# HKUST-Aerial-Robotics/A-LOAM

Hardware: AMD Instinct MI355X
Metric: HDL-64 scans/sec (whole node) (higher is better)
Workload: dtype f32 features / f64 solve

## Files before the change

a-loam_amd/csrc/aloam_device.hpp:

```cpp
#pragma once
#include <hip/hip_runtime.h>
#include <stdint.h>
#include "aloam_atan.hpp"

namespace aloam {

constexpr int kFrontSlots = 128 + 8;
constexpr int kBlockPts = 1024;
constexpr int kMaxRings = 128;
constexpr int kSectors = 6;
constexpr int kSharpPerSector = 2;
constexpr int kLessSharpPerSector = 20;
constexpr int kFlatPerSector = 4;
constexpr int kSharpPerRing = kSectors * kSharpPerSector;
constexpr int kLessSharpPerRing = kSectors * kLessSharpPerSector;
constexpr int kFlatPerRing = kSectors * kFlatPerSector;
constexpr int kNnTile = 1024;

enum ErrBits { kErrEmpty = 1, kErrRingCap = 2, kErrPointCap = 4, kErrInternal = 8 };

struct alignas(16) SeqMeta {
  int n_in;
  int first_kept, last_kept;
  int half_idx;
  float start_ori, end_ori;
  int n_cloud;
  int err;
  int n_sharp, n_less_sharp, n_flat, n_less_flat;
  int n_corner_last, n_surf_last;
  int parity;
  int pad1;
};

struct alignas(16) OdomState {
  double para_q[4];
  double para_t[3];
  double q_w[4];
  double t_w[3];
  int corner_corr[2], plane_corr[2];
  int lm_iterations[2], lm_successful[2];
  double initial_cost[2], final_cost[2];
  int termination[2];
  int inited;
  int pad;
};

enum SeqBits { kSeqActive = 1, kSeqSolve = 2, kSeqMapGrow = 4 };
__device__ __forceinline__ bool seq_idle(const int* active, int b, int bit = kSeqActive) { return active && !(active[b] & bit); }

struct EdgeRec { float cp[3], a[3], b[3]; int valid; int pad[2]; };
struct PlaneRec { float cp[3], j[3], l[3], m[3]; int valid; int pad[3]; };

struct RegArgs {
  const char* in;
  long long seq_stride;
  int pt_stride;
  int B, cap, R, NB;
  int ring_from_field;
  float min_range;
  SeqMeta* meta;
  float4* slabs;
  int slab;
  unsigned long long* front_lb;
  int* front_ticket;
  int* ringstart;
  float4* cloud;
  float* curv;
  int8_t* label;
  unsigned long long* lookback;
  unsigned epoch;
  int* ring_ticket;
  int store_debug;
  float4* sharp;
  float4* less_sharp[2];
  float4* flat;
  float4* less_flat[2];
  const int* active;
};

constexpr int kRangeRowTables = 6;
struct RangeArgs {
  const int* n_cols;
  const float2* az_xy;
  const float* row_tab;
  int rows, n_az, row_major;
  float range_scale;
};

struct OdomArgs {
  int B, cap, R;
  SeqMeta* meta;
  OdomState* state;
  const float4* sharp;
  const float4* flat;
  const float4* less_sharp[2];
  const float4* less_flat[2];
  const int* active;
  float4* grid_sorted3[2][2];
  float4* grid_sorted2[2][2];
  int* grid_start3[2][2];
  int* grid_start2[2][2];
  float4* grid_sorted3c[2][2];
  int* grid_start3c[2][2];
  int* grid_flags[2][2];
  int* grid_walk[2][2];
  int grid_H_corner, grid_H_surf;
  float4* sel_sharp;
  float4* sel_flat;
  EdgeRec* edges;
  PlaneRec* planes;
  int outer;
  int last_outer;
  int lm_max_iterations;
  int distortion;
};

template <typename T>
__device__ __forceinline__ T* row_of(T* const (&buf)[2], int k, int b, long long per) { return (k ? buf[1] : buf[0]) + b * per; }
__device__ __forceinline__ const float4* corner_last(const OdomArgs& a, int b, int parity) { return row_of(a.less_sharp, parity ^ 1, b, (long long)a.R * kLessSharpPerRing); }
__device__ __forceinline__ const float4* surf_last(const OdomArgs& a, int b, int parity) { return row_of(a.less_flat, parity ^ 1, b, (long long)a.cap); }

struct GridView {
  int H;
  float4 *sorted3, *sorted2, *sorted3c;
  int *start3, *start2, *start3c, *flags, *walk;
};
template <typename T>
__device__ __forceinline__ T* grid_ptr(T* const (&buf)[2][2], int set, int which) {
  return set ? (which ? buf[1][1] : buf[1][0]) : (which ? buf[0][1] : buf[0][0]);
}
__device__ __forceinline__ GridView grid_view(const OdomArgs& a, int b, int which, int set) {
  GridView g;
  g.H = which == 0 ? a.grid_H_corner : a.grid_H_surf;
  const long long per = which == 0 ? (long long)a.R * kLessSharpPerRing : (long long)a.cap;
  g.sorted3 = grid_ptr(a.grid_sorted3, set, which) + b * per;
  g.sorted2 = grid_ptr(a.grid_sorted2, set, which) + b * per;
  g.start3 = grid_ptr(a.grid_start3, set, which) + (long long)b * (g.H + 1);
  g.start2 = grid_ptr(a.grid_start2, set, which) + (long long)b * (g.H + 1);
  g.sorted3c = grid_ptr(a.grid_sorted3c, set, which) + b * per;
  g.start3c = grid_ptr(a.grid_start3c, set, which) + (long long)b * (g.H + 1);
  g.flags = grid_ptr(a.grid_flags, set, which) + b * 4;
  g.walk = grid_ptr(a.grid_walk, set, which) + (long long)b * 2 * (a.R + 8);
  return g;
}

__device__ __forceinline__ float4 load_point(const char* base, long long i, int stride) {
  const float* p = reinterpret_cast<const float*>(base + i * (long long)stride);
  if ((stride & 15) == 0) return *reinterpret_cast<const float4*>(p);
  if (stride == 12) return make_float4(p[0], p[1], p[2], 0.f);
  return make_float4(p[0], p[1], p[2], p[3]);
}

__device__ __forceinline__ bool point_kept(const float4& p, float thres) {
  if (!(isfinite(p.x) && isfinite(p.y) && isfinite(p.z))) return false;
  const float r2 = p.x * p.x + p.y * p.y + p.z * p.z;
  return !(r2 < thres * thres);
}

__device__ __forceinline__ double shfl_down_f64(double v, int d) {
  int lo = __double2loint(v), hi = __double2hiint(v);
  lo = __shfl_down(lo, d, 64);
  hi = __shfl_down(hi, d, 64);
  return __hiloint2double(hi, lo);
}

template <int D>
__device__ __forceinline__ unsigned xor_lane_u32(unsigned v, int lane) {
  if constexpr (D == 1) return (unsigned)__builtin_amdgcn_mov_dpp((int)v, 0xB1, 0xF, 0xF, true);
  else if constexpr (D == 2) return (unsigned)__builtin_amdgcn_mov_dpp((int)v, 0x4E, 0xF, 0xF, true);
  else {
    const unsigned up = (unsigned)__builtin_amdgcn_mov_dpp((int)v, 0x100 + D, 0xF, 0xF, true);
    const unsigned dn = (unsigned)__builtin_amdgcn_mov_dpp((int)v, 0x110 + D, 0xF, 0xF, true);
    return (lane & D) ? dn : up;
  }
}
template <int D, bool MAX>
__device__ __forceinline__ unsigned long long row_step_u64(unsigned long long v, int lane) {
  const unsigned lo = xor_lane_u32<D>((unsigned)v, lane), hi = xor_lane_u32<D>((unsigned)(v >> 32), lane);
  const unsigned long long o = ((unsigned long long)hi << 32) | lo;
  return MAX ? (o > v ? o : v) : (o < v ? o : v);
}
template <bool MAX>
__device__ __forceinline__ unsigned long long wave_extreme_u64(unsigned long long v, int lane) {
  v = row_step_u64<1, MAX>(v, lane);
  v = row_step_u64<2, MAX>(v, lane);
  v = row_step_u64<4, MAX>(v, lane);
  v = row_step_u64<8, MAX>(v, lane);
  unsigned long long best = MAX ? 0ull : ~0ull;
#pragma unroll
  for (int q = 0; q < 4; ++q) {
    const unsigned lo = (unsigned)__builtin_amdgcn_readlane((int)(unsigned)v, 16 * q), hi = (unsigned)__builtin_amdgcn_readlane((int)(unsigned)(v >> 32), 16 * q);
    const unsigned long long o = ((unsigned long long)hi << 32) | lo;
    best = MAX ? (o > best ? o : best) : (o < best ? o : best);
  }
  return best;
}

template <bool MAX>
__device__ __forceinline__ unsigned wave_reduce_u32(unsigned v) {
  constexpr int identity = MAX ? 0 : -1;
  auto op = [](unsigned a, unsigned b) { return MAX ? (a > b ? a : b) : (a < b ? a : b); };
  v = op(v, (unsigned)__builtin_amdgcn_update_dpp(identity, (int)v, 0x111, 0xF, 0xF, false));
  v = op(v, (unsigned)__builtin_amdgcn_update_dpp(identity, (int)v, 0x112, 0xF, 0xF, false));
  v = op(v, (unsigned)__builtin_amdgcn_update_dpp(identity, (int)v, 0x114, 0xF, 0xF, false));
  v = op(v, (unsigned)__builtin_amdgcn_update_dpp(identity, (int)v, 0x118, 0xF, 0xF, false));
  v = op(v, (unsigned)__builtin_amdgcn_update_dpp(identity, (int)v, 0x142, 0xA, 0xF, false));
  v = op(v, (unsigned)__builtin_amdgcn_update_dpp(identity, (int)v, 0x143, 0xC, 0xF, false));
  return (unsigned)__builtin_amdgcn_readlane((int)v, 63);
}
__device__ __forceinline__ unsigned long long wave_min_packed(unsigned long long v) {
  const unsigned hi = (unsigned)(v >> 32), lo = (unsigned)v;
  const unsigned mh = wave_reduce_u32<false>(hi);
  const unsigned long long tie = __ballot(hi == mh);
  unsigned ml;
  if (__popcll(tie) == 1) ml = (unsigned)__builtin_amdgcn_readlane((int)lo, __ffsll((long long)tie) - 1);
  else ml = wave_reduce_u32<false>(hi == mh ? lo : 0xffffffffu);
  return ((unsigned long long)mh << 32) | ml;
}

template <bool MAX>
__device__ __forceinline__ int wave_scan_i32(int v) {
  constexpr int identity = MAX ? (int)0x80000000 : 0;
  auto op = [](int a, int b) { return MAX ? (a > b ? a : b) : a + b; };
  v = op(v, __builtin_amdgcn_update_dpp(identity, v, 0x111, 0xF, 0xF, false));
  v = op(v, __builtin_amdgcn_update_dpp(identity, v, 0x112, 0xF, 0xF, false));
  v = op(v, __builtin_amdgcn_update_dpp(identity, v, 0x114, 0xF, 0xF, false));
  v = op(v, __builtin_amdgcn_update_dpp(identity, v, 0x118, 0xF, 0xF, false));
  v = op(v, __builtin_amdgcn_update_dpp(identity, v, 0x142, 0xA, 0xF, false));
  v = op(v, __builtin_amdgcn_update_dpp(identity, v, 0x143, 0xC, 0xF, false));
  return v;
}

template <typename T, int NT>
__device__ __forceinline__ T block_exclusive_scan(T v, T* lds, T* total) {
  const int tid = threadIdx.x;
  lds[tid] = v;
  __syncthreads();
  for (int d = 1; d < NT; d <<= 1) {
    const T add = tid >= d ? lds[tid - d] : T(0);
    __syncthreads();
    lds[tid] += add;
    __syncthreads();
  }
  const T incl = lds[tid];
  *total = lds[NT - 1];
  __syncthreads();
  return incl - v;
}

__device__ __forceinline__ void wave_box_reduce(float (&mn)[3], float (&mx)[3]) {
#pragma unroll
  for (int q = 0; q < 3; ++q)
    for (int d = 32; d > 0; d >>= 1) { mn[q] = fminf(mn[q], __shfl_down(mn[q], d, 64)); mx[q] = fmaxf(mx[q], __shfl_down(mx[q], d, 64)); }
}

__device__ __forceinline__ int pow2ceil(int v) { int p = 1; while (p < v) p <<= 1; return p; }
template <typename K>
__device__ __forceinline__ void bitonic_cx(K& a, K& b) {
  const K lo = a < b ? a : b, hi = a < b ? b : a;
  a = lo; b = hi;
}
template <bool FIRST, typename K>
__device__ __forceinline__ void bitonic_groups_of_eight(K* keys, int n, int tid) {
  constexpr K kInf = (K)~(K)0;
  for (int g = tid * 8; g < n; g += 2048) {
    K v[8];
#pragma unroll
    for (int u = 0; u < 8; ++u) v[u] = g + u < n ? keys[g + u] : kInf;
    if (FIRST) {
#pragma unroll
      for (int b = 0; b < 8; b += 2) bitonic_cx(v[b], v[b + 1]);
#pragma unroll
      for (int b = 0; b < 8; b += 4) { bitonic_cx(v[b], v[b + 3]); bitonic_cx(v[b + 1], v[b + 2]); }
#pragma unroll
      for (int b = 0; b < 8; b += 2) bitonic_cx(v[b], v[b + 1]);
#pragma unroll
      for (int o = 0; o < 4; ++o) bitonic_cx(v[o], v[7 - o]);
    } else {
#pragma unroll
      for (int o = 0; o < 4; ++o) bitonic_cx(v[o], v[o + 4]);
    }
#pragma unroll
    for (int b = 0; b < 8; b += 4) { bitonic_cx(v[b], v[b + 2]); bitonic_cx(v[b + 1], v[b + 3]); }
#pragma unroll
    for (int b = 0; b < 8; b += 2) bitonic_cx(v[b], v[b + 1]);
#pragma unroll
    for (int u = 0; u < 8; ++u) if (g + u < n) keys[g + u] = v[u];
  }
  __syncthreads();
}
template <typename K>
__device__ __forceinline__ void bitonic_sort_keys(K* keys, int n, int tid) {
  const int npad = pow2ceil(n);
  bitonic_groups_of_eight<true, K>(keys, n, tid);
  for (int k = 16; k <= npad; k <<= 1) {
    const int hk = k >> 1;
    for (int t = tid; t < (npad >> 1); t += 256) {
      const int base = (t / hk) * k, off = t & (hk - 1);
      const int i = base + off, l = base + (k - 1 - off);
      if (l < n) {
        const K x = keys[i], y = keys[l];
        if (x > y) { keys[i] = y; keys[l] = x; }
      }
    }
    __syncthreads();
    for (int j = k >> 2; j > 4; j >>= 1) {
      for (int t = tid; t < (npad >> 1); t += 256) {
        const int i = ((t & ~(j - 1)) << 1) | (t & (j - 1));
        const int l = i + j;
        if (l < n) {
          const K x = keys[i], y = keys[l];
          if (x > y) { keys[i] = y; keys[l] = x; }
        }
      }
      __syncthreads();
    }
    bitonic_groups_of_eight<false, K>(keys, n, tid);
  }
}
__device__ __forceinline__ void bitonic_sort_u64(unsigned long long* keys, int n, int tid) { bitonic_sort_keys<unsigned long long>(keys, n, tid); }


}
```

a-loam_amd/csrc/registration_kernels.hip:

```cpp
#include "aloam_device.hpp"
#include "registration_kernels.hpp"
#include "voxel_device.hpp"

namespace aloam {

struct RecordLoader {
  static constexpr bool kKeepPoint = true;
  const char* in; int stride;
  __device__ __forceinline__ float4 operator()(int i) const { return load_point(in, i, stride); }
};

#ifndef ALOAM_RANGE_KEEP_POINT
#define ALOAM_RANGE_KEEP_POINT 0
#endif
struct RangeLoader {
  static constexpr bool kKeepPoint = ALOAM_RANGE_KEEP_POINT;
  const unsigned short* az; const unsigned short* range;
  const float2* az_xy; const float* tab;
  unsigned div, magic; int n_az; bool row_major; float scale;
  __device__ __forceinline__ float4 operator()(int i) const {
#ifdef ALOAM_RANGE_PHASES
    asm volatile("; ##PHASE decode");
#endif
    const unsigned code = range[i];
    unsigned q = __umulhi((unsigned)i, magic), r = (unsigned)i - q * div;
    if (r >= div) { r -= div; ++q; }
    const int row = (int)(row_major ? q : r), col = (int)(row_major ? r : q);
    const int azc = az[col];
    const bool hit = code != 0u && azc < n_az;
    int ac = azc + reinterpret_cast<const int*>(tab)[4 * kMaxRings + row];
    ac = ac < 0 ? ac + n_az : ac;
    ac = ac >= n_az ? ac - n_az : ac;
    const float2 cs = az_xy[hit ? ac : 0];
    const float rho = (float)code * scale + tab[2 * kMaxRings + row];
    const float rxy = rho * tab[0 * kMaxRings + row];
    const float nan = __builtin_nanf("");
#ifdef ALOAM_RANGE_PHASES
    asm volatile("; ##PHASE body");
#endif
    return make_float4(hit ? rxy * cs.x : nan, hit ? rxy * cs.y : nan, hit ? rho * tab[1 * kMaxRings + row] + tab[3 * kMaxRings + row] : nan, tab[5 * kMaxRings + row]);
  }
};
__device__ __forceinline__ RangeLoader range_loader(const RegArgs& a, const RangeArgs& d, int b, float* tab) {
  for (int q = threadIdx.x; q < kRangeRowTables * kMaxRings; q += blockDim.x) tab[q] = d.row_tab[q];
  __syncthreads();
  const int n_cols = d.n_cols[b];
  const unsigned short* blob = reinterpret_cast<const unsigned short*>(a.in + (long long)b * a.seq_stride);
  const unsigned div = (unsigned)(d.row_major ? n_cols : d.rows);
  return RangeLoader{blob, blob + ((n_cols + 7) & ~7), d.az_xy, tab, div, div ? 0xffffffffu / div : 0u, d.n_az, d.row_major != 0, d.range_scale};
}

template <class Loader>
__device__ __forceinline__ void find_ends_body(const RegArgs& a, const int b, const int n, const Loader& load) {
  const int tid = threadIdx.x;
  __shared__ int s_first, s_last;
  if (tid == 0) { s_first = 0x7fffffff; s_last = -1; }
  __syncthreads();
  for (int base = 0; base < n; base += 4096) {
    bool any = false;
#pragma unroll
    for (int k = 0; k < 4; ++k) {
      const int i = base + k * 1024 + tid;
      if (i < n && point_kept(load(i), a.min_range)) { atomicMin(&s_first, i); any = true; }
    }
    if (__syncthreads_or(any)) break;
  }
  for (int base = 0; base < n; base += 4096) {
    bool any = false;
#pragma unroll
    for (int k = 0; k < 4; ++k) {
      const int i = n - 1 - (base + k * 1024 + tid);
      if (i >= 0 && point_kept(load(i), a.min_range)) { atomicMax(&s_last, i); any = true; }
    }
    if (__syncthreads_or(any)) break;
  }
  __syncthreads();
  if (tid == 0) {
    SeqMeta m = a.meta[b];
    m.n_in = n;
    m.first_kept = s_first;
    m.last_kept = s_last;
    m.half_idx = 0x7fffffff;
    m.err = 0;
    m.n_cloud = 0;
    m.start_ori = 0.f;
    m.end_ori = 0.f;
    if (s_last < 0) {
      m.err = kErrEmpty;
    } else {
      const float4 p0 = load(s_first);
      const float4 p1 = load(s_last);
      const float startOri = -atan2f_port(p0.y, p0.x);
      float endOri = (float)((double)(-atan2f_port(p1.y, p1.x)) + 2 * M_PI);
      if ((double)(endOri - startOri) > 3 * M_PI) endOri = (float)((double)endOri - 2 * M_PI);
      else if ((double)(endOri - startOri) < M_PI) endOri = (float)((double)endOri + 2 * M_PI);
      m.start_ori = startOri;
      m.end_ori = endOri;
    }
    if (n > a.cap) m.err |= kErrPointCap;
    a.meta[b] = m;
  }
}
__global__ __launch_bounds__(1024) void k_find_ends(RegArgs a, const int* __restrict__ n_in) {
  const int b = blockIdx.x;
  if (seq_idle(a.active, b)) return;
  find_ends_body(a, b, n_in[b], RecordLoader{a.in + (long long)b * a.seq_stride, a.pt_stride});
}

__device__ __forceinline__ int ring_from_angle(float angle, int R) {
  int scanID;
  if (R == 16) {
    scanID = (int)((double)((angle + 15) / 2) + 0.5);
    return (scanID > R - 1 || scanID < 0) ? -1 : scanID;
  }
  if (R == 32) {
    scanID = (int)(((double)angle + 92.0 / 3.0) * 3.0 / 4.0);
    return (scanID > R - 1 || scanID < 0) ? -1 : scanID;
  }
  if ((double)angle >= -8.83) scanID = (int)((double)(2 - angle) * 3.0 + 0.5);
  else scanID = R / 2 + (int)((-8.83 - (double)angle) * 2.0 + 0.5);
  if ((double)angle > 2 || (double)angle < -24.33 || scanID > 50 || scanID < 0) return -1;
  return scanID;
}
__device__ __forceinline__ int ring_of(const float4& p, int R, int ring_from_field) {
  if (ring_from_field) {
    const int scanID = (int)p.w;
    return (scanID > R - 1 || scanID < 0) ? -1 : scanID;
  }
  const float s2 = p.x * p.x + p.y * p.y;
  {
    const float t = p.z * __frsqrt_rn(s2), u = t * t;
    const float poly = 1.0f + u * (-0.3333319425582886f + u * (0.19994600117206573f + u * (-0.1420508623123169f + u * (0.10522426664829254f + u * (-0.06763934344053268f + u * 0.025188861414790154f)))));
    const float fast = t * poly * 57.29577951f;
    const int lo = ring_from_angle(fast - 2e-4f, R), hi = ring_from_angle(fast + 2e-4f, R);
    if (lo == hi && fabsf(t) <= 0.65f) return lo;
  }
  const float angle = (float)(atan((double)p.z / sqrt((double)s2)) * 180 / M_PI);
  return ring_from_angle(angle, R);
}

constexpr int kGatherSpinLimit = 1 << 20;
__device__ __forceinline__ void front_publish(unsigned long long* g, unsigned epoch, unsigned prefix, int value) {
  __hip_atomic_store(g, ((unsigned long long)((epoch << 1) | prefix) << 32) | (unsigned)value, __ATOMIC_RELAXED, __HIP_MEMORY_SCOPE_AGENT);
}
template <bool MIN>
__device__ __forceinline__ int front_lookback(unsigned long long* slot0, int blk, unsigned epoch, int local, int* err) {
  constexpr int identity = MIN ? 0x7fffffff : 0;
  unsigned long long* mine = slot0 + (long long)blk * kFrontSlots;
  if (blk == 0) { front_publish(mine, epoch, 1u, local); return identity; }
  front_publish(mine, epoch, 0u, local);
  int acc = identity;
  for (int t = blk - 1; t >= 0; --t) {
    unsigned long long g;
    int spins = 0;
    while ((unsigned)((g = __hip_atomic_load(slot0 + (long long)t * kFrontSlots, __ATOMIC_RELAXED, __HIP_MEMORY_SCOPE_AGENT)) >> 33) != (epoch & 0x7fffffffu)) {
      if (++spins > kGatherSpinLimit) { atomicOr(err, kErrInternal); g = (1ull << 32) | (unsigned)identity; break; }
      __builtin_amdgcn_s_sleep(1);
    }
    const int v = (int)(unsigned)g;
    acc = MIN ? (v < acc ? v : acc) : acc + v;
    if ((g >> 32) & 1ull) break;
  }
  front_publish(mine, epoch, 1u, MIN ? (local < acc ? local : acc) : acc + local);
  return acc;
}

template <bool FIELD_RING, class MakeLoader>
__device__ __forceinline__ void front_body(const RegArgs& a, const MakeLoader& make_loader) {
  const int b = blockIdx.x, tid = threadIdx.x, lane = tid & 63, wave = tid >> 6;
  __shared__ int s_cnt[16][kMaxRings];
  __shared__ int s_half, s_ticket;
  if (seq_idle(a.active, b)) return;
  if (tid == 0) { s_ticket = atomicAdd(a.front_ticket + b, 1); s_half = 0x7fffffff; }
  for (int q = tid; q < 16 * kMaxRings; q += 256) (&s_cnt[0][0])[q] = 0;
  __syncthreads();
  const int blk = s_ticket;
  const SeqMeta m = a.meta[b];
  const int n = m.n_in < a.cap ? m.n_in : a.cap;
  if (blk * kBlockPts >= n) return;
  const auto load = make_loader(b);
  const float startOri = m.start_ori, endOri = m.end_ori;
  int ring[4], rank[4];
  float4 p[4];
  float ori[4];
  int myhalf = 0x7fffffff;
#pragma unroll
  for (int k = 0; k < 4; ++k) {
    const int i = blk * kBlockPts + k * 256 + tid;
    ring[k] = -1;
    p[k] = make_float4(0.f, 0.f, 0.f, 0.f);
    ori[k] = 0.f;
    if (i < n) {
      const float4 q = load(i);
      if (point_kept(q, a.min_range)) {
        ring[k] = ring_of(q, a.R, FIELD_RING ? 1 : a.ring_from_field);
        if (ring[k] >= 0) {
          if constexpr (decltype(load)::kKeepPoint) p[k] = q;
          ori[k] = -atan2f_port(q.y, q.x);
          float o1 = ori[k];
          if ((double)o1 < (double)startOri - M_PI / 2) o1 = (float)((double)o1 + 2 * M_PI);
          else if ((double)o1 > (double)startOri + M_PI * 3 / 2) o1 = (float)((double)o1 - 2 * M_PI);
          if ((double)(o1 - startOri) > M_PI && i < myhalf) myhalf = i;
        }
      }
    }
  }
#pragma unroll
  for (int k = 0; k < 4; ++k) {
    rank[k] = 0;
    unsigned long long todo = __ballot(ring[k] >= 0);
    while (todo) {
      const int leader = __ffsll((long long)todo) - 1;
      const int r = __shfl(ring[k], leader, 64);
      const unsigned long long same = __ballot(ring[k] == r);
      if (ring[k] == r) rank[k] = __popcll(same & ((1ull << lane) - 1ull));
      if (lane == leader) s_cnt[k * 4 + wave][r] = __popcll(same);
      todo &= ~same;
    }
  }
  for (int d = 32; d > 0; d >>= 1) { const int o = __shfl_down(myhalf, d, 64); myhalf = o < myhalf ? o : myhalf; }
  if (lane == 0 && myhalf != 0x7fffffff) atomicMin(&s_half, myhalf);
  __syncthreads();
  unsigned long long* lb = a.front_lb + (long long)b * a.NB * kFrontSlots;
  if (tid < a.R) {
    int total = 0;
#pragma unroll
    for (int q = 0; q < 16; ++q) total += s_cnt[q][tid];
    int run = front_lookback<false>(lb + tid, blk, a.epoch, total, &a.meta[b].err);
#pragma unroll
    for (int q = 0; q < 16; ++q) { const int c = s_cnt[q][tid]; s_cnt[q][tid] = run; run += c; }
  } else if (tid == 192) {
    const int before = front_lookback<true>(lb + a.R, blk, a.epoch, s_half, &a.meta[b].err);
    s_half = before < s_half ? before : s_half;
  }
  __syncthreads();
  const int half_idx = s_half;
  float4* slabs = a.slabs + (long long)b * a.R * a.slab;
#pragma unroll
  for (int k = 0; k < 4; ++k) {
    if (ring[k] < 0) continue;
    const int i = blk * kBlockPts + k * 256 + tid;
    const int pos = s_cnt[k * 4 + wave][ring[k]] + rank[k];
    float o = ori[k];
    if (i <= half_idx) {
      if ((double)o < (double)startOri - M_PI / 2) o = (float)((double)o + 2 * M_PI);
      else if ((double)o > (double)startOri + M_PI * 3 / 2) o = (float)((double)o - 2 * M_PI);
    } else {
      o = (float)((double)o + 2 * M_PI);
      if ((double)o < (double)endOri - M_PI * 3 / 2) o = (float)((double)o + 2 * M_PI);
      else if ((double)o > (double)endOri + M_PI / 2) o = (float)((double)o - 2 * M_PI);
    }
    const float relTime = (o - startOri) / (endOri - startOri);
    const float inten = (float)((double)ring[k] + 0.1 * (double)relTime);
    float4 pk = p[k];
    if constexpr (!decltype(load)::kKeepPoint) pk = load(i);
    if (pos < a.slab) slabs[(long long)ring[k] * a.slab + pos] = make_float4(pk.x, pk.y, pk.z, inten);
  }
}
__global__ __launch_bounds__(256) __attribute__((amdgpu_waves_per_eu(8))) void k_front(RegArgs a) {
  front_body<false>(a, [&](int b) { return RecordLoader{a.in + (long long)b * a.seq_stride, a.pt_stride}; });
}
__global__ __launch_bounds__(64) void k_ring_starts(RegArgs a) {
  const int b = blockIdx.x, lane = threadIdx.x;
  if (seq_idle(a.active, b)) return;
  const int n = a.meta[b].n_in < a.cap ? a.meta[b].n_in : a.cap;
  const int nb = (n + kBlockPts - 1) / kBlockPts;
  const unsigned long long* last = a.front_lb + ((long long)b * a.NB + (nb > 0 ? nb - 1 : 0)) * kFrontSlots;
  int run = 0, err = 0;
  for (int base = 0; base < a.R; base += 64) {
    const int r = base + lane;
    int c = 0;
    if (r < a.R && nb > 0) {
      const unsigned long long g = last[r];
      if ((unsigned)(g >> 32) != (((a.epoch & 0x7fffffffu) << 1) | 1u)) err |= kErrInternal; else c = (int)(unsigned)g;
      if (c > a.slab) { c = a.slab; err |= kErrRingCap; }
    }
    const int inc = wave_scan_i32<false>(c);
    if (r < a.R) a.ringstart[b * (a.R + 1) + r] = run + inc - c;
    run += __builtin_amdgcn_readlane(inc, 63);
  }
  if (err) atomicOr(&a.meta[b].err, err);
  if (lane == 0) {
    a.ringstart[b * (a.R + 1) + a.R] = run;
    a.meta[b].n_cloud = run;
    int half = 0x7fffffff;
    if (nb > 0) { const unsigned long long g = last[a.R]; if ((unsigned)(g >> 32) == (((a.epoch & 0x7fffffffu) << 1) | 1u)) half = (int)(unsigned)g; }
    a.meta[b].half_idx = half;
    a.front_ticket[b] = 0;
  }
}

__global__ __launch_bounds__(256) void k_dense_cloud(RegArgs a) {
  const int r = blockIdx.x, b = blockIdx.y;
  if (seq_idle(a.active, b)) return;
  const int start = a.ringstart[b * (a.R + 1) + r], n = a.ringstart[b * (a.R + 1) + r + 1] - start;
  const float4* src = a.slabs + ((long long)b * a.R + r) * a.slab;
  float4* dst = a.cloud + (long long)b * a.cap + start;
  for (int i = threadIdx.x; i < n; i += 256) dst[i] = src[i];
}

template <bool MAX>
__device__ __forceinline__ unsigned wave_extreme_u32(unsigned v, int lane) { (void)lane; return wave_reduce_u32<MAX>(v); }

__device__ __forceinline__ void publish_count(unsigned long long* slot, unsigned epoch, int count) {
  __hip_atomic_store(slot, ((unsigned long long)epoch << 32) | (unsigned)count, __ATOMIC_RELAXED, __HIP_MEMORY_SCOPE_AGENT);
}
__device__ __forceinline__ int gather_counts(const unsigned long long* slots, int upto, unsigned epoch, int lane, int* err) {
  int sum = 0;
  for (int base = 0; base < upto; base += 64) {
    const int q = base + lane;
    if (q < upto) {
      unsigned long long g;
      int spins = 0;
      while ((unsigned)((g = __hip_atomic_load(slots + q, __ATOMIC_RELAXED, __HIP_MEMORY_SCOPE_AGENT)) >> 32) != epoch) {
        if (++spins > kGatherSpinLimit) { atomicOr(err, kErrInternal); g = 0; break; }
        __builtin_amdgcn_s_sleep(1);
      }
      sum += (int)(unsigned)g;
    }
  }
  sum = wave_scan_i32<false>(sum);
  return __builtin_amdgcn_readlane(sum, 63);
}
constexpr unsigned kCurvThresholdBits = 0x3DCCCCCDu;
constexpr unsigned kInfBits = 0x7f800000u;
template <int K6>
__device__ __forceinline__ void pick_sector(int j, unsigned init_marks, int L, int lane, const float* curv_l, const unsigned char* flags,
                                            short* s_pick, int* s_misc) {
  constexpr int kSlots = kSharpPerSector + kLessSharpPerSector + kFlatPerSector;
  constexpr int NRP = (K6 + 3) / 4;
  const int sp = (L * j) / 6, len = (L * (j + 1)) / 6 - sp;
  const int first = sp + 5;
  typedef unsigned keys_t __attribute__((ext_vector_type(16)));
  static_assert(K6 <= 16, "sector registers");
  keys_t cc;
  unsigned rp[NRP];
#pragma unroll
  for (int q = 0; q < NRP; ++q) rp[q] = 0;
#pragma unroll
  for (int r = 0; r < K6; ++r) {
    const int pos = r * 64 + lane;
    cc[r] = 0u;
    if (pos < len) {
      const int i = first + pos;
      rp[r / 4] |= (unsigned)(flags[i] >> 2) << (8 * (r % 4));
      if (!(pos < 5 && ((init_marks >> pos) & 1u))) cc[r] = __float_as_uint(curv_l[i]) + 1u;
    }
  }
  unsigned spill = 0;
  auto kill = [&](int kr, int f, const unsigned dead) {
    unsigned rb;
    if constexpr (NRP <= 2) {
      const unsigned r0 = (unsigned)__builtin_amdgcn_readlane((int)rp[0], f), r1 = (unsigned)__builtin_amdgcn_readlane((int)rp[NRP - 1], f);
      rb = (unsigned)((((unsigned long long)r1 << 32) | r0) >> (8 * kr));
    } else {
      unsigned rpk = (unsigned)__builtin_amdgcn_readlane((int)rp[0], f);
#pragma unroll
      for (int q = 1; q < NRP; ++q) { const unsigned x = (unsigned)__builtin_amdgcn_readlane((int)rp[q], f); if (q == (kr >> 2)) rpk = x; }
      rb = rpk >> (8 * (kr & 3));
    }
    const int fw = (int)(rb & 7u), bk = (int)((rb >> 3) & 7u);
    const int P = kr * 64 + f;
    const int lo = f - bk, w = fw + bk;
    {
      const bool in = (unsigned)(lane - lo) <= (unsigned)w;
      const unsigned old = cc[kr];
      cc[kr] = in ? dead : old;
    }
    if ((unsigned)lo > (unsigned)(63 - w)) {
      asm volatile("");
      if (lo < 0 && kr > 0) { asm volatile(""); const bool in = lane >= 64 + lo; const unsigned old = cc[kr - 1]; cc[kr - 1] = in ? dead : old; }
      if (lo >= 0 && kr + 1 < K6) { asm volatile(""); const bool in = lane <= lo + w - 64; const unsigned old = cc[kr + 1]; cc[kr + 1] = in ? dead : old; }
    }
    if (P + 5 >= len) {
      asm volatile("");
      const int e = P + fw - (len - 1);
      if (e > 0) spill |= (1u << e) - 1u;
    }
    return P;
  };
  int picks = 0;
  int count = 0;
  for (; count < kLessSharpPerSector; ++count) {
    unsigned m = cc[0];
#pragma unroll
    for (int r = 1; r < K6; ++r) m = cc[r] > m ? cc[r] : m;
    int krl = 0;
#pragma unroll
    for (int r = 1; r < K6; ++r) krl = cc[r] == m ? r : krl;
    const unsigned cmax = wave_reduce_u32<true>(m);
    if (!(cmax - 1u >= kCurvThresholdBits && cmax - 1u <= kInfBits)) break;
    const unsigned long long tie = __ballot(m == cmax);
    int f = __builtin_ctzll(tie);
    int kr = __builtin_amdgcn_readlane(krl, f);
    if (__popcll(tie) != 1) {
      asm volatile("");
      const unsigned w = wave_reduce_u32<true>(m == cmax ? (unsigned)(krl * 64 + lane) : 0u);
      f = (int)(w & 63u); kr = (int)(w >> 6);
    }
    const int P = kill(kr, f, 0u);
    picks = lane == count ? first + P : picks;
  }
  const int ncorner = count;
  if (lane < ncorner) s_pick[j * kSlots + kSharpPerSector + lane] = (short)picks;
#pragma unroll
  for (int r = 0; r < K6; ++r) cc[r] -= 1u;
  count = 0;
  while (true) {
    unsigned m = cc[0];
#pragma unroll
    for (int r = 1; r < K6; ++r) m = cc[r] < m ? cc[r] : m;
    int krl = K6 - 1;
#pragma unroll
    for (int r = K6 - 2; r >= 0; --r) krl = cc[r] == m ? r : krl;
    const unsigned cmin = wave_reduce_u32<false>(m);
    if (!(cmin < kCurvThresholdBits)) break;
    const unsigned long long tie = __ballot(m == cmin);
    int f = __builtin_ctzll(tie);
    int kr = __builtin_amdgcn_readlane(krl, f);
    if (__popcll(tie) != 1) {
      asm volatile("");
      const unsigned w = wave_reduce_u32<false>(m == cmin ? (unsigned)(krl * 64 + lane) : 0xffffffffu);
      f = (int)(w & 63u); kr = (int)(w >> 6);
    }
    picks = lane == count ? first + kr * 64 + f : picks;
    ++count;
    if (count >= kFlatPerSector) break;
    kill(kr, f, 0xffffffffu);
  }
  if (lane < count) s_pick[j * kSlots + kSharpPerSector + kLessSharpPerSector + lane] = (short)picks;
  if (lane == 0) { s_misc[1 + j] = ncorner | (count << 8); s_misc[8 + j] = (int)spill; }
}


#ifdef ALOAM_PHASE_CLOCK
__device__ unsigned long long g_phase_clock[2][32];
constexpr int phase_slot(const char* s) { unsigned h = 0; while (*s) h = h * 33u + (unsigned char)*s++; return (int)(h % 32u); }
#define ALOAM_PHASE(name) do { asm volatile("; ##PHASE " name); if (threadIdx.x == 0) { constexpr int slot_ = phase_slot(name); \
    atomicAdd(&g_phase_clock[0][slot_], (unsigned long long)__builtin_readcyclecounter()); atomicAdd(&g_phase_clock[1][slot_], 1ull); } } while (0)
#else
#define ALOAM_PHASE(name) asm volatile("; ##PHASE " name)
#endif
__device__ __forceinline__ bool label_is_member(unsigned char f) { return ((f + 1u) & 2u) == 0u; }
__device__ __forceinline__ int label_of(unsigned char f) { const int c = f & 3; return c == 3 ? -1 : c; }
template <int NPAD, typename K, int SHIFT>
__device__ __forceinline__ int voxel_runs_tail(unsigned char* smem, unsigned char* flags, int* s_scan, int* s_misc,
                                               const float4* cloud, float4* out, int L, int tid, int lane, int wave,
                                               unsigned long long* lb_lf, int ring, int nrings, unsigned epoch, int* err) {
  const unsigned* vis = reinterpret_cast<const unsigned*>(smem);
  K* rkeys = reinterpret_cast<K*>(smem);
  constexpr unsigned kEMask = SHIFT >= 32 ? 0xffffffffu : ((1u << (SHIFT & 31)) - 1u);
  constexpr int EIT = NPAD / 256;
  unsigned hmask = 0;
  int hrank[EIT];
  unsigned myvi[EIT];
#pragma unroll
  for (int it = 0; it < EIT; ++it) {
    const int e = it * 256 + tid;
    bool h = false;
    myvi[it] = 0xffffffffu;
    if (e < L) {
      const unsigned vi = vis[e];
      const unsigned char fe = flags[e + 5];
      const bool member = label_is_member(fe);
      h = member && (e == 0 || !label_is_member(flags[e + 4]) || vis[e - 1] != vi);
      myvi[it] = vi;
      flags[e + 5] = (unsigned char)((fe & 3u) | (member && !h ? 4u : 0u));
    }
    const unsigned long long m = __ballot(h);
    hrank[it] = __popcll(m & ((1ull << lane) - 1ull));
    if (h) hmask |= 1u << it;
    if (lane == 0) s_scan[it * 4 + wave] = __popcll(m);
  }
  __syncthreads();
  static_assert(4 * EIT <= 64, "one wave scans the table");
  if (wave == 0) {
    const int c = lane < 4 * EIT ? s_scan[lane] : 0;
    const int inc = wave_scan_i32<false>(c);
    if (lane < 4 * EIT) s_scan[lane] = inc - c;
    if (lane == 63) s_scan[64] = inc;
  }
  __syncthreads();
  const int n_runs = s_scan[64];
#pragma unroll
  for (int it = 0; it < EIT; ++it) hrank[it] += s_scan[it * 4 + wave];
#pragma unroll
  for (int it = 0; it < EIT; ++it)
    if ((hmask >> it) & 1u) { const int e = it * 256 + tid; rkeys[hrank[it]] = (K)(((K)myvi[it] << SHIFT) | (K)e); }
  __syncthreads();
  ALOAM_PHASE("after_run_heads");
  bitonic_sort_keys<K>(rkeys, n_runs, tid);

  ALOAM_PHASE("after_sort");
  int n_vox = 0;
  unsigned vmask = 0;
  int vrank[EIT];
  __syncthreads();
#pragma unroll
  for (int it = 0; it < EIT; ++it) {
    const int p = it * 256 + tid;
    const bool h = p < n_runs && (p == 0 || (unsigned)(rkeys[p - 1] >> SHIFT) != (unsigned)(rkeys[p] >> SHIFT));
    const unsigned long long m = __ballot(h);
    vrank[it] = __popcll(m & ((1ull << lane) - 1ull));
    if (h) vmask |= 1u << it;
    if (lane == 0) s_scan[it * 4 + wave] = __popcll(m);
  }
  __syncthreads();
  if (wave == 0) {
    const int c = lane < 4 * EIT ? s_scan[lane] : 0;
    const int inc = wave_scan_i32<false>(c);
    if (lane < 4 * EIT) s_scan[lane] = inc - c;
    if (lane == 63) { s_scan[64] = inc; publish_count(lb_lf + ring, epoch, inc); }
  }
  __syncthreads();
  n_vox = s_scan[64];
#pragma unroll
  for (int it = 0; it < EIT; ++it) vrank[it] += s_scan[it * 4 + wave];
  if (wave == 0) {
    const unsigned long long* lb0 = lb_lf - 3 * nrings;
    const int b0 = gather_counts(lb0 + 0 * nrings, ring, epoch, lane, err), b1 = gather_counts(lb0 + 1 * nrings, ring, epoch, lane, err);
    const int b2 = gather_counts(lb0 + 2 * nrings, ring, epoch, lane, err), b3 = gather_counts(lb_lf, ring, epoch, lane, err);
    if (lane == 0) { s_misc[40] = b0; s_misc[41] = b1; s_misc[42] = b2; s_misc[43] = b3; }
  }
  __syncthreads();
  ALOAM_PHASE("after_vox_heads_gather");
  out += s_misc[43];
#pragma unroll
  for (int it = 0; it < EIT; ++it) {
    if (!((vmask >> it) & 1u)) continue;
    const int p = it * 256 + tid;
    const unsigned vi = (unsigned)(rkeys[p] >> SHIFT);
    voxel::Centroid c;
    for (int q = p; q < n_runs; ++q) {
      const K kq = rkeys[q];
      if ((unsigned)(kq >> SHIFT) != vi) break;
      int e = (int)((unsigned)kq & kEMask);
      bool more;
      do {
        const float4 p0 = cloud[e + 5], p1 = cloud[e + 6], p2 = cloud[e + 7], p3 = cloud[e + 8];
        const bool c1 = e + 1 < L && (flags[e + 6] & 4), c2 = e + 2 < L && (flags[e + 7] & 4), c3 = e + 3 < L && (flags[e + 8] & 4);
        more = e + 4 < L && (flags[e + 9] & 4);
        c.add(p0);
        if (!c1) break;
        c.add(p1);
        if (!c2) break;
        c.add(p2);
        if (!c3) break;
        c.add(p3);
        e += 4;
      } while (more);
    }
    out[vrank[it]] = c.get();
  }
  ALOAM_PHASE("after_centroids");
  return n_vox;
}

template <int NPAD>
__global__ __launch_bounds__(256) __attribute__((amdgpu_waves_per_eu(NPAD <= 2048 ? 8 : 4))) void k_ring_features(RegArgs a, float leaf) {
  constexpr int MAXN = NPAD + 11;
  constexpr int ITEMS = (MAXN + 255) / 256;
  const int b = blockIdx.x, tid = threadIdx.x, lane = tid & 63, wave = tid >> 6;
  extern __shared__ __attribute__((aligned(16))) unsigned char smem_ticket[];
  int* s_ticket = reinterpret_cast<int*>(smem_ticket);
  typedef __attribute__((address_space(1))) int global_int;
  if (seq_idle(a.active, b)) return;
  if (tid == 0) *s_ticket = __hip_atomic_fetch_add((global_int*)(a.ring_ticket + b), 1, __ATOMIC_RELAXED, __HIP_MEMORY_SCOPE_AGENT);
  __syncthreads();
  int r_ = __builtin_amdgcn_readfirstlane(*s_ticket);
  asm volatile("" : "+s"(r_));
  const int r = r_;
  __syncthreads();
  if (r >= a.R) {
    if (tid == 0) atomicOr(&a.meta[b].err, kErrInternal);
    return;
  }
  const int start = a.ringstart[b * (a.R + 1) + r];
  const int n = a.ringstart[b * (a.R + 1) + r + 1] - start;
  unsigned long long* lb = a.lookback + (long long)b * 4 * a.R;
  if (n - 11 < 6 || n > MAXN) {
    if (n - 11 >= 6 && tid == 0) atomicOr(&a.meta[b].err, kErrRingCap);
    if (tid < 4) publish_count(lb + tid * a.R + r, a.epoch, 0);
    return;
  }

  extern __shared__ __attribute__((aligned(16))) unsigned char smem[];
  ALOAM_PHASE("ticket_taken");
  constexpr int A_BYTES = 8 * NPAD + 128;
  constexpr int TW = 256 + 10;
  static_assert(2 * 3 * TW * 4 <= A_BYTES && 4 * MAXN <= A_BYTES, "region A holds the curvature tiles and the curvature array");
  typedef float f2 __attribute__((ext_vector_type(2)));
  f2 (*txy)[TW] = reinterpret_cast<f2 (*)[TW]>(smem);
  float (*tz)[TW] = reinterpret_cast<float (*)[TW]>(smem + 2 * TW * 8);
  constexpr int FLAG_BYTES = (MAXN + 15) & ~15;
  unsigned char* flags = smem + ((A_BYTES + 15) & ~15);
  int* s_scan = reinterpret_cast<int*>(smem + ((A_BYTES + 15) & ~15) + FLAG_BYTES);
  float (*s_red)[4] = reinterpret_cast<float (*)[4]>(s_scan + 256);
  int* s_misc = reinterpret_cast<int*>(s_scan + 256 + 24);
  constexpr int kSlots = kSharpPerSector + kLessSharpPerSector + kFlatPerSector;
  short* s_pick = reinterpret_cast<short*>(s_misc + 48);

  constexpr int CELLS_OFF = (4 * MAXN + 15) & ~15;
  static_assert(CELLS_OFF + 4 * MAXN <= A_BYTES, "the packed cells sit behind the curvature array in region A");
  unsigned* cells = reinterpret_cast<unsigned*>(smem + CELLS_OFF);
  const float inv = voxel::inverse_leaf(leaf);
  unsigned long long* gapw = reinterpret_cast<unsigned long long*>(s_scan);
  static_assert((ITEMS * 4 + 2) * 8 <= 256 * 4, "the gap bits fit the scan scratch");
  if (tid == 0) { s_misc[44] = 0; gapw[0] = ~0ull; gapw[ITEMS * 4 + 1] = ~0ull; }
  const float4* cloud = a.slabs + ((long long)b * a.R + r) * a.slab;
  const int L = n - 11;
  float cv[ITEMS];
  const float4 zero4 = make_float4(0.f, 0.f, 0.f, 0.f);
  float4 pa = tid - 5 >= 0 && tid - 5 < n ? cloud[tid - 5] : zero4, pb = tid < 10 && tid + 251 < n ? cloud[tid + 251] : zero4;
  unsigned oxy[2] = {(unsigned)tid * 8u, (unsigned)tid * 8u + TW * 8u}, oz[2] = {2u * TW * 8u + (unsigned)tid * 4u, 2u * TW * 8u + TW * 4u + (unsigned)tid * 4u};
  asm volatile("" : "+v"(oxy[1]), "+v"(oz[0]), "+v"(oz[1]));
  txy[0][tid] = f2{pa.x, pa.y}; tz[0][tid] = pa.z;
  if (tid < 10) { txy[0][tid + 256] = f2{pb.x, pb.y}; tz[0][tid + 256] = pb.z; }
  __syncthreads();
#pragma unroll
  for (int it = 0; it < ITEMS; ++it) {
    const int i = tid + it * 256;
    const bool more = (it + 1) * 256 < n;
    if (more) {
      const int ia = i + 251, ib = i + 507;
      pa = ia < n ? cloud[ia] : zero4;
      pb = tid < 10 && ib < n ? cloud[ib] : zero4;
    }
    cv[it] = 0.f;
    bool gapf = true;
    if (i < n) {
      const f2* q = reinterpret_cast<const f2*>(smem + oxy[it & 1]) + 5;
      const float* zs = reinterpret_cast<const float*>(smem + oz[it & 1]) + 5;
      const f2 q0 = q[0];
      const float z0 = zs[0];
      if (i < n - 1) {
        const f2 d = q[1] - q0, dd = d * d;
        const float dz = zs[1] - z0;
        gapf = (double)(dd.x + dd.y + dz * dz) > 0.05;
      }
      if (i >= 5 && i < n - 5) {
        f2 sxy = q[-5] + q[-4]; sxy = sxy + q[-3]; sxy = sxy + q[-2]; sxy = sxy + q[-1]; sxy = sxy - 10.f * q0;
        sxy = sxy + q[1]; sxy = sxy + q[2]; sxy = sxy + q[3]; sxy = sxy + q[4]; sxy = sxy + q[5];
        const float dZ = zs[-5] + zs[-4] + zs[-3] + zs[-2] + zs[-1] - 10 * z0 + zs[1] + zs[2] + zs[3] + zs[4] + zs[5];
        const f2 ss = sxy * sxy;
        cv[it] = ss.x + ss.y + dZ * dZ;
        if (a.store_debug) a.curv[(long long)b * a.cap + start + i] = cv[it];
      }
      const f2 cxy = q0 * inv;
      const float fx = floorf(cxy.x), fy = floorf(cxy.y), fz = floorf(z0 * inv);
      const bool okc = voxel::cell_packable(fx, fy, fz);
      if (!okc) s_misc[44] = 1;
      cells[i] = okc ? voxel::pack_cell(fx, fy, fz) : 0u;
    }
    {
      const unsigned long long gb = __ballot(gapf);
      if (lane == 0) gapw[1 + it * 4 + wave] = gb;
    }
    if (more) {
      const int nb = (it + 1) & 1;
      txy[nb][tid] = f2{pa.x, pa.y}; tz[nb][tid] = pa.z;
      if (tid < 10) { txy[nb][tid + 256] = f2{pb.x, pb.y}; tz[nb][tid + 256] = pb.z; }
    }
    __syncthreads();
  }

  ALOAM_PHASE("after_curvature");
  float* curv_l = reinterpret_cast<float*>(smem);
  {
    const unsigned* gw32 = reinterpret_cast<const unsigned*>(gapw);
#pragma unroll
    for (int it = 0; it < ITEMS; ++it) {
      const int i = tid + it * 256;
      if (i < n) {
        const unsigned bit = (unsigned)i + 59u;
        const unsigned win = __builtin_amdgcn_alignbit(gw32[(bit >> 5) + 1], gw32[bit >> 5], bit & 31u);
        const int fw = __builtin_ctz((win >> 5) | 32u);
        const int bk = __builtin_ctz(__builtin_bitreverse32(win << 27) | 32u);
        curv_l[i] = cv[it];
        flags[i] = (unsigned char)((fw << 2) | (bk << 5));
      }
    }
  }
  __syncthreads();

  ALOAM_PHASE("after_reach");
  constexpr int K6 = (NPAD / 6 + 2 + 63) / 64;
#pragma unroll 1
  for (int j = __builtin_amdgcn_readfirstlane(wave); j < kSectors; j += 4) pick_sector<K6>(j, 0u, L, lane, curv_l, flags, s_pick, s_misc);
  __syncthreads();
  ALOAM_PHASE("after_select1");
  if (wave == 0) {
    unsigned carry = (unsigned)s_misc[8];
#pragma unroll 1
    for (int j = 1; j < kSectors; ++j) {
      const int sp = (L * j) / 6, len = (L * (j + 1)) / 6 - sp;
      const unsigned m = len >= 5 ? carry : (carry & ((1u << len) - 1u));
      if (m) {
        const int nc = s_misc[1 + j] & 0xff, nfl = s_misc[1 + j] >> 8;
        bool hit = false;
        if (lane < kSlots) {
          const int slot = lane;
          const bool used = slot >= kSharpPerSector && (slot < kSharpPerSector + kLessSharpPerSector ? slot - kSharpPerSector < nc : slot - kSharpPerSector - kLessSharpPerSector < nfl);
          if (used) { const int pos = s_pick[j * kSlots + slot] - 5 - sp; hit = pos < 5 && ((m >> pos) & 1u); }
        }
        if (__ballot(hit)) pick_sector<K6>(j, m, L, lane, curv_l, flags, s_pick, s_misc);
      }
      carry = (len >= 5 ? 0u : (carry >> len)) | (unsigned)s_misc[8 + j];
    }
  }
  __syncthreads();
  if (tid < kSectors * kSlots) {
    const int j = tid / kSlots, slot = tid % kSlots;
    const int nc = s_misc[1 + j] & 0xff, nfl = s_misc[1 + j] >> 8;
    if (slot >= kSharpPerSector) {
      if (slot < kSharpPerSector + kLessSharpPerSector) { const int q = slot - kSharpPerSector; if (q < nc) flags[s_pick[j * kSlots + slot]] = q < kSharpPerSector ? 2 : 1; }
      else { const int q = slot - kSharpPerSector - kLessSharpPerSector; if (q < nfl) flags[s_pick[j * kSlots + slot]] = 3; }
    }
  }
  __syncthreads();
  if (wave == 0) {
    int nc = 0, nf = 0;
    if (lane < kSectors) { nc = s_misc[1 + lane] & 0xff; nf = s_misc[1 + lane] >> 8; }
    const int ns = nc < kSharpPerSector ? nc : kSharpPerSector;
    const int is = wave_scan_i32<false>(ns), il = wave_scan_i32<false>(nc), ifl = wave_scan_i32<false>(nf);
    if (lane < kSectors) { s_misc[16 + lane] = is - ns; s_misc[24 + lane] = il - nc; s_misc[32 + lane] = ifl - nf; }
    if (lane == 0) {
      publish_count(lb + 0 * a.R + r, a.epoch, __builtin_amdgcn_readlane(is, 63));
      publish_count(lb + 1 * a.R + r, a.epoch, __builtin_amdgcn_readlane(il, 63));
      publish_count(lb + 2 * a.R + r, a.epoch, __builtin_amdgcn_readlane(ifl, 63));
    }
  }

  ALOAM_PHASE("after_redo_labels_counts");
  if (a.store_debug) for (int i = tid; i < n; i += 256) a.label[(long long)b * a.cap + start + i] = (int8_t)label_of(flags[i]);

  unsigned* vis = reinterpret_cast<unsigned*>(smem);
  static_assert(8 * NPAD <= A_BYTES, "region A holds the voxel indices, then the run keys");
  bool overflow = false;
  long long cells_in_box = 0;
  bool voxels_done = false;
  int (*s_redi)[4] = reinterpret_cast<int (*)[4]>(s_red);
  if (s_misc[44] == 0) {
    int mn[3] = {0x7fffffff, 0x7fffffff, 0x7fffffff}, mx[3] = {(int)0x80000000, (int)0x80000000, (int)0x80000000};
    for (int e = tid; e < L; e += 256) {
      const int i = e + 5;
      if (label_is_member(flags[i])) {
        int c[3];
        voxel::unpack_cell(cells[i], c);
        mn[0] = min(mn[0], c[0]); mx[0] = max(mx[0], c[0]); mn[1] = min(mn[1], c[1]); mx[1] = max(mx[1], c[1]); mn[2] = min(mn[2], c[2]); mx[2] = max(mx[2], c[2]);
      }
    }
#pragma unroll
    for (int q = 0; q < 3; ++q) {
      mn[q] = (int)(wave_reduce_u32<false>((unsigned)mn[q] ^ 0x80000000u) ^ 0x80000000u);
      mx[q] = (int)(wave_reduce_u32<true>((unsigned)mx[q] ^ 0x80000000u) ^ 0x80000000u);
      if (lane == 0) { s_redi[q][wave] = mn[q]; s_redi[3 + q][wave] = mx[q]; }
    }
    __syncthreads();
#pragma unroll
    for (int q = 0; q < 3; ++q) {
      mn[q] = min(min(s_redi[q][0], s_redi[q][1]), min(s_redi[q][2], s_redi[q][3]));
      mx[q] = max(max(s_redi[3 + q][0], s_redi[3 + q][1]), max(s_redi[3 + q][2], s_redi[3 + q][3]));
    }
    __syncthreads();
    voxel::PackedBox box;
    if (voxel::make_packed_box(mn, mx, box)) {
      cells_in_box = voxel::box_cells(box.divc);
      for (int e = tid; e < L; e += 256) {
        const int i = e + 5;
        unsigned vi = 0xffffffffu;
        if (label_is_member(flags[i])) vi = voxel::packed_cell_index(box, cells[i]);
        vis[e] = vi;
      }
      voxels_done = true;
    }
  }
  if (!voxels_done) {
    float mn[3] = {3.4e38f, 3.4e38f, 3.4e38f}, mx[3] = {-3.4e38f, -3.4e38f, -3.4e38f};
    for (int e = tid; e < L; e += 256) {
      const int i = e + 5;
      if (label_is_member(flags[i])) {
        const float4 p = cloud[i];
        mn[0] = fminf(mn[0], p.x); mx[0] = fmaxf(mx[0], p.x);
        mn[1] = fminf(mn[1], p.y); mx[1] = fmaxf(mx[1], p.y);
        mn[2] = fminf(mn[2], p.z); mx[2] = fmaxf(mx[2], p.z);
      }
    }
    wave_box_reduce(mn, mx);
#pragma unroll
    for (int q = 0; q < 3; ++q)
      if (lane == 0) { s_red[q][wave] = mn[q]; s_red[3 + q][wave] = mx[q]; }
    __syncthreads();
    float gmn[3], gmx[3];
#pragma unroll
    for (int q = 0; q < 3; ++q) {
      gmn[q] = fminf(fminf(s_red[q][0], s_red[q][1]), fminf(s_red[q][2], s_red[q][3]));
      gmx[q] = fmaxf(fmaxf(s_red[3 + q][0], s_red[3 + q][1]), fmaxf(s_red[3 + q][2], s_red[3 + q][3]));
    }
    const voxel::Box box = voxel::make_box(gmn, gmx, inv);
    overflow = box.unfiltered;
    cells_in_box = voxel::box_cells(box.divb);
    for (int e = tid; e < L; e += 256) {
      const int i = e + 5;
      unsigned vi = 0xffffffffu;
      if (label_is_member(flags[i])) {
        if (overflow) vi = (unsigned)e;
        else {
          const float4 p = cloud[i];
          vi = voxel::cell_index(box, p.x, p.y, p.z, inv);
        }
      }
      vis[e] = vi;
    }
  }
  __syncthreads();
  ALOAM_PHASE("after_bbox_voxidx");
  constexpr int EB = NPAD <= 2048 ? 11 : 12;
  const int parity = a.meta[b].parity;
  float4* out = row_of(a.less_flat, parity, b, a.cap);
  if (overflow || cells_in_box <= (1ll << (32 - EB))) {
    voxel_runs_tail<NPAD, unsigned, EB>(smem, flags, s_scan, s_misc, cloud, out, L, tid, lane, wave, lb + 3 * a.R, r, a.R, a.epoch, &a.meta[b].err);
  } else
    voxel_runs_tail<NPAD, unsigned long long, 32>(smem, flags, s_scan, s_misc, cloud, out, L, tid, lane, wave, lb + 3 * a.R, r, a.R, a.epoch, &a.meta[b].err);
  {
    const int base_sharp = s_misc[40], base_less = s_misc[41], base_flat = s_misc[42];
    static_assert(kSectors * kSlots <= 256, "one thread per pick slot");
    if (const int q = tid; q < kSectors * kSlots) {
      const int j = q / kSlots, slot = q % kSlots;
      const int ncorner = s_misc[1 + j] & 0xff, nflat = s_misc[1 + j] >> 8;
      if (slot < kSharpPerSector) {
        if (slot < ncorner) a.sharp[(long long)b * a.R * kSharpPerRing + base_sharp + s_misc[16 + j] + slot] = cloud[s_pick[j * kSlots + kSharpPerSector + slot]];
      } else if (slot < kSharpPerSector + kLessSharpPerSector) {
        const int k = slot - kSharpPerSector;
        if (k < ncorner) row_of(a.less_sharp, parity, b, (long long)a.R * kLessSharpPerRing)[base_less + s_misc[24 + j] + k] = cloud[s_pick[j * kSlots + slot]];
      } else {
        const int k = slot - kSharpPerSector - kLessSharpPerSector;
        if (k < nflat) a.flat[(long long)b * a.R * kFlatPerRing + base_flat + s_misc[32 + j] + k] = cloud[s_pick[j * kSlots + slot]];
      }
    }
  }
  ALOAM_PHASE("picks_out");
}

__global__ __launch_bounds__(64) void k_cloud_sizes(RegArgs a) {
  const int b = blockIdx.x, lane = threadIdx.x;
  if (seq_idle(a.active, b)) return;
  const unsigned long long* lb = a.lookback + (long long)b * 4 * a.R;
  int* err = &a.meta[b].err;
  const int n0 = gather_counts(lb + 0 * a.R, a.R, a.epoch, lane, err), n1 = gather_counts(lb + 1 * a.R, a.R, a.epoch, lane, err);
  const int n2 = gather_counts(lb + 2 * a.R, a.R, a.epoch, lane, err), n3 = gather_counts(lb + 3 * a.R, a.R, a.epoch, lane, err);
  if (lane == 0) { a.meta[b].n_sharp = n0; a.meta[b].n_less_sharp = n1; a.meta[b].n_flat = n2; a.meta[b].n_less_flat = n3; a.ring_ticket[b] = 0; }
}

__global__ __launch_bounds__(1024) void k_find_ends_range(RegArgs a, RangeArgs d) {
  const int b = blockIdx.x;
  __shared__ float s_tab[kRangeRowTables * kMaxRings];
  if (seq_idle(a.active, b)) return;
  find_ends_body(a, b, d.n_cols[b] * d.rows, range_loader(a, d, b, s_tab));
}

__global__ __launch_bounds__(256) __attribute__((amdgpu_waves_per_eu(8))) void k_front_range(RegArgs a, RangeArgs d) {
  __shared__ float s_tab[kRangeRowTables * kMaxRings];
  if (seq_idle(a.active, blockIdx.x)) return;
  front_body<true>(a, [&](int b) { return range_loader(a, d, b, s_tab); });
}

size_t ring_features_lds_bytes(int npad) {
  const int maxn = npad + 11;
  const int a_bytes = 8 * npad + 128;
  const int flag_bytes = (maxn + 15) & ~15;
  return (size_t)((a_bytes + 15) & ~15) + (size_t)flag_bytes + (256 + 24 + 48) * sizeof(int) + 6 * 26 * sizeof(short) + 8;
}

void launch_find_ends(const RegArgs& a, const int* d_nin, hipStream_t s) { hipLaunchKernelGGL(k_find_ends, dim3(a.B), dim3(1024), 0, s, a, d_nin); }
void launch_front(const RegArgs& a, hipStream_t s) { hipLaunchKernelGGL(k_front, dim3(a.B, a.NB), dim3(256), 0, s, a); }
void launch_find_ends_range(const RegArgs& a, const RangeArgs& d, hipStream_t s) { hipLaunchKernelGGL(k_find_ends_range, dim3(a.B), dim3(1024), 0, s, a, d); }
void launch_front_range(const RegArgs& a, const RangeArgs& d, hipStream_t s) { hipLaunchKernelGGL(k_front_range, dim3(a.B, a.NB), dim3(256), 0, s, a, d); }
void launch_ring_starts(const RegArgs& a, hipStream_t s) { hipLaunchKernelGGL(k_ring_starts, dim3(a.B), dim3(64), 0, s, a); }
void launch_dense_cloud(const RegArgs& a, hipStream_t s) { hipLaunchKernelGGL(k_dense_cloud, dim3(a.R, a.B), dim3(256), 0, s, a); }
void launch_ring_features(const RegArgs& a, int npad, float leaf, hipStream_t s) {
  const size_t lds = ring_features_lds_bytes(npad);
  if (npad <= 2048) hipLaunchKernelGGL(k_ring_features<2048>, dim3(a.B, a.R), dim3(256), lds, s, a, leaf);
  else hipLaunchKernelGGL(k_ring_features<4096>, dim3(a.B, a.R), dim3(256), lds, s, a, leaf);
  hipLaunchKernelGGL(k_cloud_sizes, dim3(a.B), dim3(64), 0, s, a);
}

}

#ifdef ALOAM_PHASE_CLOCK
extern "C" int aloam_debug_phase_clock(unsigned long long* out) { return (int)hipMemcpyFromSymbol(out, HIP_SYMBOL(aloam::g_phase_clock), sizeof(unsigned long long) * 64); }
#endif
```

Measured before the change: 132,700.

## Use blocked register bitonic sort processing eight keys per thread per pass

Adds a bitonic sort variant in which each thread loads eight strided keys into registers and performs up to three compare-exchange stages before writing back. Each merge level then needs fewer shared-memory round trips and __syncthreads barriers, and the voxel run-head sort now calls this variant. The cost is more registers per thread and a more complex index scheme, with padding handled through infinity sentinels.

```diff
diff --git a/a-loam_amd/csrc/aloam_device.hpp b/a-loam_amd/csrc/aloam_device.hpp
--- a/a-loam_amd/csrc/aloam_device.hpp
+++ b/a-loam_amd/csrc/aloam_device.hpp
@@ -320,5 +320,69 @@
 }
 __device__ __forceinline__ void bitonic_sort_u64(unsigned long long* keys, int n, int tid) { bitonic_sort_keys<unsigned long long>(keys, n, tid); }
 
-
-}
+template <int S, int STAGES, bool FIRST, int CAP, typename K>
+__device__ __forceinline__ void bitonic_pass_of_eight(K* keys, int n, int tid) {
+  constexpr K kInf = (K)~(K)0;
+  constexpr int U = 8 * S <= CAP ? 8 : CAP / S;
+  for (int q = tid; (q & ~(S - 1)) * 8 < n; q += 256) {
+    const int i0 = (q & ~(S - 1)) * 8 + (q & (S - 1));
+    K* p = keys + i0;
+    K v[8];
+#pragma unroll
+    for (int u = 0; u < 8; ++u) v[u] = u < U ? p[u * S] : kInf;
+#pragma unroll
+    for (int u = 0; u < U; ++u) if (i0 + u * S >= n) v[u] = kInf;
+    if (FIRST) {
+#pragma unroll
+      for (int b = 0; b < 8; b += 2) bitonic_cx(v[b], v[b + 1]);
+#pragma unroll
+      for (int b = 0; b < 8; b += 4) { bitonic_cx(v[b], v[b + 3]); bitonic_cx(v[b + 1], v[b + 2]); }
+#pragma unroll
+      for (int b = 0; b < 8; b += 2) bitonic_cx(v[b], v[b + 1]);
+#pragma unroll
+      for (int o = 0; o < 4; ++o) bitonic_cx(v[o], v[7 - o]);
+    } else if (STAGES == 3) {
+#pragma unroll
+      for (int o = 0; o < 4; ++o) bitonic_cx(v[o], v[o + 4]);
+    }
+    if (STAGES >= 2) {
+#pragma unroll
+      for (int b = 0; b < 8; b += 4) { bitonic_cx(v[b], v[b + 2]); bitonic_cx(v[b + 1], v[b + 3]); }
+    }
+#pragma unroll
+    for (int b = 0; b < 8; b += 2) bitonic_cx(v[b], v[b + 1]);
+#pragma unroll
+    for (int u = 0; u < U; ++u) p[u * S] = v[u];
+  }
+  __syncthreads();
+}
+template <int S, int CAP, typename K>
+__device__ __forceinline__ void bitonic_level(K* keys, int n, int tid, int stages) {
+  if (stages >= 3) bitonic_pass_of_eight<S, 3, false, CAP, K>(keys, n, tid);
+  else if (stages == 2) bitonic_pass_of_eight<S, 2, false, CAP, K>(keys, n, tid);
+  else if (stages == 1) bitonic_pass_of_eight<S, 1, false, CAP, K>(keys, n, tid);
+}
+template <typename K, int CAP>
+__device__ __forceinline__ void bitonic_sort_blocked(K* keys, int n, int tid) {
+  static_assert(CAP >= 512 && CAP <= 4096 && (CAP & (CAP - 1)) == 0, "levels S = 1, 8, 64 (and 512 from 2048 keys on)");
+  const int npad = pow2ceil(n);
+  bitonic_pass_of_eight<1, 3, true, CAP, K>(keys, n, tid);
+  for (int lk = 4; (1 << lk) <= npad; ++lk) {
+    const int k = 1 << lk, hk = k >> 1;
+    for (int t = tid; t < (npad >> 1); t += 256) {
+      const int off = t & (hk - 1), i = ((t - off) << 1) + off, l = i + (k - 1 - 2 * off);
+      if (l < n) {
+        const K x = keys[i], y = keys[l];
+        if (x > y) { keys[i] = y; keys[l] = x; }
+      }
+    }
+    __syncthreads();
+    if constexpr (CAP >= 2048) bitonic_level<512, CAP, K>(keys, n, tid, lk - 10);
+    bitonic_level<64, CAP, K>(keys, n, tid, lk - 7);
+    bitonic_level<8, CAP, K>(keys, n, tid, lk - 4);
+    bitonic_pass_of_eight<1, 3, false, CAP, K>(keys, n, tid);
+  }
+}
+
+
+}
diff --git a/a-loam_amd/csrc/registration_kernels.hip b/a-loam_amd/csrc/registration_kernels.hip
--- a/a-loam_amd/csrc/registration_kernels.hip
+++ b/a-loam_amd/csrc/registration_kernels.hip
@@ -489,7 +489,7 @@
     if ((hmask >> it) & 1u) { const int e = it * 256 + tid; rkeys[hrank[it]] = (K)(((K)myvi[it] << SHIFT) | (K)e); }
   __syncthreads();
   ALOAM_PHASE("after_run_heads");
-  bitonic_sort_keys<K>(rkeys, n_runs, tid);
+  bitonic_sort_blocked<K, NPAD>(rkeys, n_runs, tid);
 
   ALOAM_PHASE("after_sort");
   int n_vox = 0;
```

Result: faster. 134,700, median of 6 (+1.5%).
